# yancie-yjr/StreamYOLO

Measured on NVIDIA B200. Metric: frame-pairs/sec StreamYOLO-l 600x960 fwd+loss, higher is better.
Workload: dtype bf16

## Files before the change

include/streamyolo_sm100.h:

```cpp
#ifndef STREAMYOLO_SM100_H_
#define STREAMYOLO_SM100_H_

#include <stddef.h>
#include <stdint.h>

#ifdef __cplusplus
extern "C" {
#endif

typedef struct CUstream_st* sy_stream_t;

enum {
  SY_OK = 0,
  SY_EINVAL = 1,
  SY_EARCH = 2,
  SY_ELAUNCH = 3,
  SY_EWORKSPACE = 4
};

typedef struct {
  void* ptr;
  int32_t n, h, w, c;
  int64_t pitch;
} SyTensor;

const char* sy_last_error_string(void);
int sy_version(void);
int sy_check_device(void);

int sy_l2_persist_window(void* ptr, size_t bytes, float hit_ratio, size_t* granted, sy_stream_t stream);

enum { SY_CONV_RAW = 0, SY_CONV_FUSED = 1 };

typedef struct {
  const float* gamma; const float* beta;
  float* running_mean; float* running_var;
  int64_t* num_batches_tracked;
  int32_t c_begin;
} SyBnSegment;

typedef struct {
  SyTensor x;
  SyTensor y;
  const void* w;
  int32_t kh, kw;
  int32_t stride;
  int32_t mode;
  int32_t act;
  const float* scale;
  const float* shift;
  SyTensor res;
  int32_t split_n;
  float* stat_partials;
  int32_t n_partials;
  int32_t* rows_written;
  SyBnSegment bn[2];
  float momentum, eps;
  float* scale_shift;
  float* mean_invstd;
  uint32_t* sync;
  SyTensor apply_y, apply_res;
  int64_t apply_y_group1_offset, apply_res_group1_offset;
  void* debug_timeline;
  int32_t debug_timeline_events;
  int32_t debug_flags;
// ... 181 lines not shown
```

streamyolo_b200/csrc/conv_simt.cu:

```cuda
#include "common.cuh"

namespace sy {

struct SimtConvParams {
  const __nv_bfloat16* x; long long x_pitch;
  const __nv_bfloat16* w;
  __nv_bfloat16* y; long long y_pitch;
  const __nv_bfloat16* res; long long res_pitch;
  const float* scale; const float* shift;
  int N, H, W, Cin, Ho, Wo, Cout, kh, kw, stride, pad_h, pad_w, mode, act;
};

__global__ void conv_simt_kernel(const SimtConvParams p) {
  const int G = p.Cout / 8;
  const long long total = (long long)p.N * p.Ho * p.Wo * G;
  for (long long idx = blockIdx.x * (long long)blockDim.x + threadIdx.x; idx < total;
       idx += (long long)gridDim.x * blockDim.x) {
    const int g = (int)(idx % G);
    const long long pix = idx / G;
    const int ox = (int)(pix % p.Wo);
    const int oy = (int)((pix / p.Wo) % p.Ho);
    const int n = (int)(pix / ((long long)p.Wo * p.Ho));
    float acc[8];
#pragma unroll
// ... 95 lines not shown
    }
#pragma unroll
    for (int i = 0; i < 16; ++i) red[threadIdx.x][i] = s[i];
    __syncthreads();
    if (pl == 0 && g < G) {
      for (int i = 0; i < 16; ++i) {
        float a = 0.f;
        for (int q = 0; q < PL; ++q) a += red[q * lanes + gl][i];
        out[(i >> 3) * C + g * 8 + (i & 7)] = a;
      }
    }
    __syncthreads();
  }
}

}

using namespace sy;

extern "C" int sy_conv2d_simt(const SyConvDesc* d, sy_stream_t stream_) {
  cudaStream_t stream = reinterpret_cast<cudaStream_t>(stream_);
  SY_REQUIRE(d != nullptr, SY_EINVAL, "null descriptor");
  const SyTensor& x = d->x;
  const SyTensor& y = d->y;
  SY_REQUIRE(view_ok(x) && view_ok(y) && d->w != nullptr, SY_EINVAL, "conv2d_simt: bad x/y view or null weights");
  SY_REQUIRE((d->kh == 1 || d->kh == 3) && (d->kw == 1 || d->kw == 3) && (d->stride == 1 || d->stride == 2), SY_EINVAL,
             "conv2d_simt: kernel %dx%d stride %d unsupported", d->kh, d->kw, d->stride);
  SimtConvParams p{};
  p.pad_h = (d->kh - 1) / 2; p.pad_w = (d->kw - 1) / 2;
  p.N = x.n; p.H = x.h; p.W = x.w; p.Cin = x.c; p.Cout = y.c; p.kh = d->kh; p.kw = d->kw; p.stride = d->stride;
  p.Ho = (x.h + 2 * p.pad_h - d->kh) / d->stride + 1;
  p.Wo = (x.w + 2 * p.pad_w - d->kw) / d->stride + 1;
  SY_REQUIRE(y.n == x.n && y.h == p.Ho && y.w == p.Wo, SY_EINVAL, "conv2d_simt: output view mismatch");
  p.x = reinterpret_cast<const __nv_bfloat16*>(x.ptr); p.x_pitch = x.pitch;
  p.w = reinterpret_cast<const __nv_bfloat16*>(d->w);
  p.y = reinterpret_cast<__nv_bfloat16*>(y.ptr); p.y_pitch = y.pitch;
  p.mode = d->mode; p.act = d->act; p.scale = d->scale; p.shift = d->shift;
  if (d->mode == SY_CONV_FUSED && d->res.ptr) {
    SY_REQUIRE(view_ok(d->res) && d->res.c == y.c && d->res.h == y.h && d->res.w == y.w && d->res.n == y.n, SY_EINVAL,
               "conv2d_simt: residual view mismatch");
    p.res = reinterpret_cast<const __nv_bfloat16*>(d->res.ptr); p.res_pitch = d->res.pitch;
  }
  const long long total = (long long)p.N * p.Ho * p.Wo * (p.Cout / 8);
  const int blocks = (int)((total + 127) / 128 < 148 * 16 ? (total + 127) / 128 : 148 * 16);
  conv_simt_kernel<<<blocks, 128, 0, stream>>>(p);
  return launch_status("conv_simt_kernel");
}

extern "C" int sy_focus_pack(const float* x, int32_t b, int32_t in_ch, int32_t h, int32_t w_px, int32_t frames,
                             SyTensor y, sy_stream_t stream_) {
  cudaStream_t stream = reinterpret_cast<cudaStream_t>(stream_);
  SY_REQUIRE(x && view_ok(y), SY_EINVAL, "focus_pack: null input or bad output view");
  SY_REQUIRE(h % 2 == 0 && w_px % 2 == 0 && frames >= 1 && frames * 3 <= in_ch, SY_EINVAL,
             "focus_pack: h=%d w=%d must be even, frames=%d in_ch=%d", h, w_px, frames, in_ch);
  SY_REQUIRE(y.n == frames * b && y.h == h / 2 && y.w == w_px / 2 && y.c == 64, SY_EINVAL,
             "focus_pack: output view must be [frames*b, h/2, w/2, 64]");
  const int rows = y.n * y.h;
  const int blocks = rows < 148 * 16 ? rows : 148 * 16;
  focus_pack_kernel<<<blocks, 256, 0, stream>>>(x, b, in_ch, h, w_px, frames, reinterpret_cast<__nv_bfloat16*>(y.ptr),
                                                y.pitch);
  return launch_status("focus_pack_kernel");
}

extern "C" int sy_stats_num_partials(int32_t n, int32_t hw) { return n * cdiv(hw, kStatChunk); }

extern "C" int sy_channel_stats(SyTensor x, float* partials, int32_t n_partials, sy_stream_t stream_) {
// ... 9 lines not shown
```

streamyolo_b200/csrc/conv_tc.cu:

```cuda
#include <cuda.h>
#include <stdio.h>

#include "common.cuh"
#include "tc_common.cuh"

namespace sy {
namespace tc {

constexpr int kBlockM = 128;
constexpr int kBlockK = 64;
constexpr int kThreads = 640;
constexpr int kEpiThreads = 256;
constexpr int kTailThreads = 512;
constexpr int kABytes = kBlockM * 128;
constexpr int kMaxStages = 8;

struct BnSeg {
  const float* gamma; const float* beta;
  float* rmean; float* rvar; long long* nbt;
  int c_begin;
};

struct Params {
  int N, Ho, Wo, Cout, Cin;
  int kh, kw, stride, pad_h, pad_w;
  int th, tw, tiles_x, tiles_y;
  int m_tiles, n_tiles, total_tiles;
  FastDiv fd_m_tiles, fd_per_img, fd_tiles_x, fd_tw;
  int m_tiles2, total_tiles2;
  FastDiv fd_m_tiles2;
  int P_total;
  int gp;
  FastDiv fd_hw, fd_wo;
  int cblocks, kblocks, stages;
  int stage_tiles;
  int team;
  int stagesA;
  int halo_pitch;
  int halo_bytes;
  int halo_tx;
  int mode, act;
  __nv_bfloat16* y;
  long long y_pitch;
  const __nv_bfloat16* res;
  long long res_pitch;
  const float* scale;
  const float* shift;
  int split_n;
  float* partials;
  int n_seg;
  BnSeg seg[2];
  float momentum, eps;
  double inv_cnt[2];
  float unbias[2];
  float* ss;
  float* mi;
  unsigned int* sync;
  __nv_bfloat16* ap_y; long long ap_y_pitch;
  const __nv_bfloat16* ap_res; long long ap_res_pitch;
  long long ap_y_goff1, ap_res_goff1;
  int ap_act;
  long long* timeline;
  int timeline_cap;
  int debug_flags;
  float* dbg_f32;
};

template <bool TL>
__device__ __forceinline__ void tl_rec(const Params& p, int& n, int role, int phase, int tile, int kb) {
  if (TL && p.timeline != nullptr && blockIdx.x == 0 && n + 1 < p.timeline_cap) {
    p.timeline[2 * n] = ((long long)role << 28) | ((long long)phase << 24) | ((long long)(tile & 0xffff) << 8) | (kb & 0xff);
    p.timeline[2 * n + 1] = clock64();
    ++n;
  }
// ... 47 lines not shown
conv_tc_kernel(const __grid_constant__ CUtensorMap tmA, const __grid_constant__ CUtensorMap tmB,
               const __grid_constant__ CUtensorMap tmY, const Params p) {
  using C = Cfg<BN>;
  constexpr bool LIN = (AM == 1);
  constexpr bool HALO = (AM == 2);
  static_assert(!PAIR || AM != 0, "pair mode: linear or halo tiles");
  constexpr int kBB = PAIR ? C::kBBytes / 2 : C::kBBytes;
  const uint32_t crank = PAIR ? cluster_ctarank() : 0u;
#define SY_T_FIRST (PAIR ? (int)(blockIdx.x >> 1) : (int)blockIdx.x)
#define SY_T_STEP (PAIR ? (int)(gridDim.x >> 1) : (int)gridDim.x)
#define SY_T_END (PAIR ? p.total_tiles2 : p.total_tiles)
  auto tile_nm = [&](int tile, int& n_tile, int& m_tile) {
    if constexpr (PAIR) {
      n_tile = fdiv(tile, p.fd_m_tiles2);
      m_tile = 2 * (tile - n_tile * p.m_tiles2) + (int)crank;
    } else {
      n_tile = fdiv(tile, p.fd_m_tiles);
      m_tile = tile - n_tile * p.m_tiles;
    }
  };
  const int S = p.stages;
  constexpr int kSub = HALO ? (BN == 256 ? 1 : 3) : (PAIR ? 2 : C::kSub);
  static_assert(!PAIR || C::kSub <= 2, "pair mode: the host sizes the ring for two sub-blocks per stage");
  extern __shared__ uint8_t smem_raw[];
  uint8_t* smem = smem_raw + ((1024u - (smem_u32(smem_raw) & 1023u)) & 1023u);
  uint8_t* sA = smem;
  uint8_t* sB = sA + (HALO ? p.stagesA * p.halo_bytes : S * kSub * kABytes);
  uint8_t* sStage = sB + S * kSub * kBB;
  uint64_t* bars = reinterpret_cast<uint64_t*>(sStage + p.stage_tiles * kSlabBytes);
  const int sflip = p.stage_tiles - 1;
  uint32_t* tmem_slot = reinterpret_cast<uint32_t*>(bars + 2 * kMaxStages + 4);
  float* sAcc = reinterpret_cast<float*>(bars + 32);
  float* sScale = sAcc;
  float* sShift = sScale + 256;

  const int warp = threadIdx.x >> 5;
  const int lane = threadIdx.x & 31;
  pdl_launch_dependents();
  int tl_k = 3 * (p.timeline_cap / 4);
  if (threadIdx.x == 16 * 32) tl_rec<TL>(p, tl_k, 4, 0, 0, 0);
  const uint32_t bar0 = smem_u32(bars);
  auto full_bar = [&](int s) { return bar0 + 8u * s; };
  auto empty_bar = [&](int s) { return bar0 + 8u * (kMaxStages + s); };
  auto tfull_bar = [&](int a) { return bar0 + 8u * (2 * kMaxStages + a); };
  auto tempty_bar = [&](int a) { return bar0 + 8u * (2 * kMaxStages + 2 + a); };
  auto fullA_bar = [&](int s) { return bar0 + 8u * (2 * kMaxStages + 6 + s); };
  auto emptyA_bar = [&](int s) { return bar0 + 8u * (2 * kMaxStages + 9 + s); };

  if (threadIdx.x == 19 * 32) {
    prefetch_tmap(&tmA);
    prefetch_tmap(&tmB);
    prefetch_tmap(&tmY);
    for (int s = 0; s < S; ++s) {
      mbar_init(full_bar(s), (HALO ? 1 : 2) * (PAIR ? 2 : 1));
      mbar_init(empty_bar(s), 1);
    }
    if (HALO) {
      for (int s = 0; s < p.stagesA; ++s) {
        mbar_init(fullA_bar(s), PAIR ? 2 : 1);
        mbar_init(emptyA_bar(s), 1);
      }
    }
    for (int a = 0; a < 2; ++a) {
      mbar_init(tfull_bar(a), 1);
      mbar_init(tempty_bar(a), PAIR ? 16 : ((p.team && BN == kSlabCols) ? kEpiThreads / 2 : kEpiThreads));
    }
    fence_barrier_init();
// ... 227 lines not shown
            if (sb0 + kSub >= p.kblocks) umma_commit_2cta(tfull_bar(acc));
          } else {
            umma_commit(empty_bar(stage));
            if (sb0 + kSub >= p.kblocks) umma_commit(tfull_bar(acc));
          }
          tl_rec<TL>(p, tl_n, 1, 3, tile, sb0);
        }
        __syncwarp();
        if (++stage == S) { stage = 0; phase ^= 1u; }
      }
    }
  } else if (warp == 16) {
    const uint32_t stage_base = smem_u32(sStage);
    int sbuf = 0, prev = -1;
    int tl_s = 7 * (p.timeline_cap / 8);
    const int nbar = p.team ? 416 : 544;
    bar_free_arrive(0, nbar);
    if (sflip) bar_free_arrive(1, nbar);
    for (int tile = SY_T_FIRST; tile < SY_T_END; tile += SY_T_STEP) {
      int n_tile, m_tile;
        tile_nm(tile, n_tile, m_tile);
      int c1, c2, c3;
      if constexpr (LIN) {
        c1 = m_tile * kBlockM; c2 = 0; c3 = 0;
      } else {
        const int img = fdiv(m_tile, p.fd_per_img), rem = m_tile - img * per_img;
        const int py = fdiv(rem, p.fd_tiles_x), px = rem - py * p.tiles_x;
        c1 = px * p.tw; c2 = py * p.th; c3 = img;
      }
      for (int slab = 0; slab < BN / kSlabCols; ++slab, sbuf ^= sflip) {
        bar_staged_wait(sbuf, nbar);
        if (lane == 0) tl_rec<TL>(p, tl_s, 6, 0, tile, slab);
        if (elect_one()) {
          tma_store_4d(&tmY, stage_base + (uint32_t)(sbuf * kSlabBytes), n_tile * BN + slab * kSlabCols, c1, c2, c3);
          bulk_commit();
          if (sflip) {
            if (prev >= 0) bulk_wait_read1();
          } else {
            bulk_wait_read();
          }
        }
        __syncwarp();
        if (lane == 0) tl_rec<TL>(p, tl_s, 6, 1, tile, slab);
        if (sflip) {
          if (prev >= 0) bar_free_arrive(prev, nbar);
          prev = sbuf;
        } else {
          bar_free_arrive(0, nbar);
        }
      }
    }
    if (sflip && prev >= 0) {
      if (elect_one()) bulk_wait_read();
      __syncwarp();
      bar_free_arrive(prev, nbar);
    }
    if (lane == 0) {
      if (p.ap_y != nullptr) {
        bulk_wait_all();
        asm volatile("fence.proxy.async;" ::: "memory");
      } else {
        bulk_wait_read();
      }
    }
    __syncwarp();
    asm volatile("bar.sync 4, 288;" ::: "memory");
  } else if (warp >= 8 && warp < 16) {
    const int ew = warp - 8;
// ... 189 lines not shown
            packed[i] = valid ? pack_bf16(__uint_as_float(v[2 * i]), __uint_as_float(v[2 * i + 1])) : 0u;
          tmem_ld32(taddr + (uint32_t)(cl + 32), v);
          tl_rec<TL>(p, tl_n, 2, 2, tile, slab);
          bar_free_wait(team, 416);
#pragma unroll
          for (int g = 0; g < 4; ++g)
            sts128(my_tile_row + ((((uint32_t)g) ^ rsw) << 4), packed[4 * g], packed[4 * g + 1], packed[4 * g + 2], packed[4 * g + 3]);
          tmem_ld_wait();
          if (slab == last) {
            tcgen05_fence_before();
            mbar_arrive(tempty_bar(acc));
          }
          if (p.dbg_f32 != nullptr && valid) {
            float* o = p.dbg_f32 + pix * p.Cout + n0 + cl + 32;
#pragma unroll
            for (int i = 0; i < 32; ++i)
              if (n0 + cl + 32 + i < p.Cout) o[i] = __uint_as_float(v[i]);
          }
#pragma unroll
          for (int i = 0; i < 16; ++i)
            packed[i] = valid ? pack_bf16(__uint_as_float(v[2 * i]), __uint_as_float(v[2 * i + 1])) : 0u;
#pragma unroll
          for (int g = 0; g < 4; ++g)
            sts128(my_tile_row + ((((uint32_t)(4 + g)) ^ rsw) << 4), packed[4 * g], packed[4 * g + 1], packed[4 * g + 2], packed[4 * g + 3]);
          fence_proxy_async();
          bar_staged_arrive(team, 416);
          tl_rec<TL>(p, tl_n, 2, 3, tile, slab);
        }
      }
      tl_epi = tl_n;
      bar_free_wait(team, 416);
      asm volatile("bar.sync 4, 288;" ::: "memory");
    } else {
    for (int tile = SY_T_FIRST; tile < SY_T_END; tile += SY_T_STEP, ++it) {
      const int acc = it & 1;
      const uint32_t acc_phase = (uint32_t)(it >> 1) & 1u;
      int n_tile, m_tile;
        tile_nm(tile, n_tile, m_tile);
      bool valid;
      long long pix;
      if constexpr (LIN) {
        pix = (long long)m_tile * kBlockM + row;
        valid = pix < p.P_total;
      } else {
        const int img = fdiv(m_tile, p.fd_per_img), rem = m_tile - img * per_img;
        const int py = fdiv(rem, p.fd_tiles_x), px = rem - py * p.tiles_x;
        const int oy = py * p.th + ty, ox = px * p.tw + tx;
        valid = in_patch && (oy < p.Ho) && (ox < p.Wo);
        pix = ((long long)img * p.Ho + oy) * p.Wo + ox;
      }
      const int n0 = n_tile * BN;
      tl_rec<TL>(p, tl_n, 2, 0, tile, 0);
      if (p.mode == SY_CONV_FUSED) {
        epi_bar();
        for (int c = et; c < BN; c += kEpiThreads) {
          const int cg = n0 + c;
          sScale[c] = (cg < p.Cout && p.scale) ? p.scale[cg] : 1.0f;
          sShift[c] = (cg < p.Cout && p.shift) ? p.shift[cg] : 0.0f;
        }
        epi_bar();
      }
      mbar_wait(tfull_bar(acc), acc_phase);
      tl_rec<TL>(p, tl_n, 2, 1, tile, 0);
      tcgen05_fence_after();
      const uint32_t taddr = tmem_base + (uint32_t)(acc * BN) + ((uint32_t)(q * 32) << 16);
      const bool pf = !(p.debug_flags & 32);
      uint32_t v[32];
      tmem_ld32(taddr + (uint32_t)(half * 32), v);
#pragma unroll 1
      for (int slab = 0; slab < BN / kSlabCols; ++slab, sbuf ^= sflip) {
        const int cl = slab * kSlabCols + half * 32;
        if (!pf && slab > 0) tmem_ld32(taddr + (uint32_t)cl, v);
        tmem_ld_wait();
        if (slab == BN / kSlabCols - 1) {
          tcgen05_fence_before();
          if constexpr (PAIR) {
            __syncwarp();
            if (lane == 0) mbar_arrive_cluster(mapa(tempty_bar(acc), 0u));
          } else {
            mbar_arrive(tempty_bar(acc));
          }
        }
        if (p.dbg_f32 != nullptr && valid) {
          float* o = p.dbg_f32 + pix * p.Cout + n0 + cl;
#pragma unroll
          for (int i = 0; i < 32; ++i)
            if (n0 + cl + i < p.Cout) o[i] = __uint_as_float(v[i]);
        }
        uint32_t packed[16];
        if (p.mode == SY_CONV_RAW) {
#pragma unroll
          for (int i = 0; i < 16; ++i)
            packed[i] = valid ? pack_bf16(__uint_as_float(v[2 * i]), __uint_as_float(v[2 * i + 1])) : 0u;
        } else {
          float f[32];
#pragma unroll
          for (int i = 0; i < 32; ++i) {
            float t = __uint_as_float(v[i]) * sScale[cl + i] + sShift[cl + i];
            f[i] = p.act ? silu_f(t) : t;
          }
          if (p.res != nullptr && valid) {
            const __nv_bfloat16* rp = p.res + pix * p.res_pitch + n0 + cl;
#pragma unroll
            for (int g = 0; g < 4; ++g) {
              if (n0 + cl + g * 8 < p.Cout) {
                const uint4 rv = *reinterpret_cast<const uint4*>(rp + g * 8);
                f[g * 8 + 0] += bf16_lo(rv.x); f[g * 8 + 1] += bf16_hi(rv.x);
                f[g * 8 + 2] += bf16_lo(rv.y); f[g * 8 + 3] += bf16_hi(rv.y);
                f[g * 8 + 4] += bf16_lo(rv.z); f[g * 8 + 5] += bf16_hi(rv.z);
                f[g * 8 + 6] += bf16_lo(rv.w); f[g * 8 + 7] += bf16_hi(rv.w);
              }
            }
          }
#pragma unroll
          for (int i = 0; i < 16; ++i) packed[i] = valid ? pack_bf16(f[2 * i], f[2 * i + 1]) : 0u;
        }
        if (pf && slab + 1 < BN / kSlabCols) tmem_ld32(taddr + (uint32_t)(cl + kSlabCols), v);
        tl_rec<TL>(p, tl_n, 2, 2, tile, slab);
        bar_free_wait(sbuf);
        const uint32_t my_tile_row = my_row + (uint32_t)(sbuf * kSlabBytes);
#pragma unroll
        for (int g = 0; g < 4; ++g) {
          const uint32_t j = (uint32_t)(half * 4 + g);
          sts128(my_tile_row + ((j ^ rsw) << 4), packed[4 * g], packed[4 * g + 1], packed[4 * g + 2], packed[4 * g + 3]);
        }
        fence_proxy_async();
        bar_staged_arrive(sbuf);
        tl_rec<TL>(p, tl_n, 2, 3, tile, slab);
        tl_rec<TL>(p, tl_n, 2, 4, tile, slab);
      }
    }
    tl_epi = tl_n;
// ... 287 lines not shown

template <int BN, int AM>
static int resident_pairs(size_t smem) {
  if constexpr (AM == 0) {
    return 0;
  } else {
    static size_t seen_smem[4] = {0, 0, 0, 0};
    static int seen_n[4] = {0, 0, 0, 0};
    for (int i = 0; i < 4; ++i)
      if (seen_smem[i] == smem) return seen_n[i];
    if (!set_smem_attr<BN, AM, true>()) return 0;
    cudaLaunchConfig_t cfg = {};
    cfg.gridDim = dim3(num_sms() & ~1);
    cfg.blockDim = dim3(kThreads);
    cfg.dynamicSmemBytes = smem;
    cudaLaunchAttribute at[1];
    at[0].id = cudaLaunchAttributeClusterDimension;
    at[0].val.clusterDim.x = 2; at[0].val.clusterDim.y = 1; at[0].val.clusterDim.z = 1;
    cfg.attrs = at;
    cfg.numAttrs = 1;
    int n = 0;
    if (cudaOccupancyMaxActiveClusters(&n, conv_tc_kernel<BN, false, AM, true>, &cfg) != cudaSuccess) {
      cudaGetLastError();
      n = 0;
    }
    for (int i = 0; i < 4; ++i)
      if (seen_smem[i] == 0) { seen_smem[i] = smem; seen_n[i] = n; break; }
    return n;
  }
}

template <int BN, int AM>
static int make_plan(Params& p, Plan* out) {
  const int acc_bytes = (p.mode == SY_CONV_RAW && p.partials) ? 16 * p.Cout : 2048;
  const double kbc = BN == 256 ? 665.0 : (BN == 128 ? 515.0 : 560.0);
  const bool main_loop_bound = !(p.kblocks * kbc < epi_cycles_per_slab(BN) * (BN / 64));
  bool pair = false;
  if (AM != 0) {
    const char* e = getenv("SY_CONV_PAIR");
    const bool off = e != nullptr && e[0] == '0', force = e != nullptr && e[0] == '1';
    const char* pa = getenv("SY_PAIR_APPLY");
    const bool pair_apply = pa != nullptr && pa[0] == '1';
    pair = !off && (force || (main_loop_bound && (p.ap_y == nullptr || pair_apply)));
  }
  for (int attempt = 0; attempt < 2; ++attempt) {
    p.stage_tiles = main_loop_bound ? 1 : 2;
    if (const char* e = getenv("SY_STAGE_TILES")) p.stage_tiles = (e[0] == '2') ? 2 : 1;
    p.team = (p.stage_tiles == 2 && p.mode == SY_CONV_RAW) ? 1 : 0;
    if (const char* e = getenv("SY_CONV_TEAM")) p.team = (e[0] != '0' && p.stage_tiles == 2 && p.mode == SY_CONV_RAW) ? 1 : 0;
    if (pair) { p.stage_tiles = 1; p.team = 0; }
    const int bbytes = Cfg<BN>::kBBytes / (pair ? 2 : 1);
    const int fixed_bytes = Cfg<BN>::kFixedBytes + (p.stage_tiles - 1) * kSlabBytes;
    int smem;
    if (AM == 2) {
      const int taps = (BN == 256) ? 1 : 3;
      p.stagesA = (BN == 64 && p.cblocks > 1) ? 3 : 2;
      int stages = (kSmemLimit - fixed_bytes - acc_bytes - p.stagesA * p.halo_bytes) / (taps * bbytes);
      if (stages > kMaxStages) stages = kMaxStages;
      SY_REQUIRE(stages >= 2, SY_EINVAL, "conv2d_tc(halo): Cout=%d leaves no room for the weight ring", p.Cout);
      p.stages = stages;
      smem = fixed_bytes + acc_bytes + p.stagesA * p.halo_bytes + stages * taps * bbytes;
    } else {
      const int ksub = pair ? 2 : Cfg<BN>::kSub;
      const int stage_bytes = ksub * (kABytes + bbytes);
      int stages = (kSmemLimit - fixed_bytes - acc_bytes) / stage_bytes;
      if (stages > kMaxStages) stages = kMaxStages;
      if ((p.debug_flags >> 8) & 15) stages = min(stages, (p.debug_flags >> 8) & 15);
// ... 114 lines not shown
  tc::EncodeTiledFn enc = tc::get_encode();
  SY_REQUIRE(enc != nullptr, SY_EARCH, "cuTensorMapEncodeTiled not available from the driver");

  tc::Params p{};
  p.debug_flags = d->debug_flags;
  if (const char* e = getenv("SY_CONV_DEBUG")) p.debug_flags |= atoi(e);
  p.N = x.n; p.Ho = ho; p.Wo = wo; p.Cout = y.c; p.Cin = x.c;
  p.kh = d->kh; p.kw = d->kw; p.stride = d->stride; p.pad_h = ph; p.pad_w = pw;
  const bool halo = d->kh == 3 && d->kw == 3 && d->stride == 1 && tc::linear_tiles() &&
                    tc::use_halo(x.n, ho, wo, y.c, 9 * cdiv(x.c, tc::kBlockK));
  const bool lin = !halo && tc::linear_tiles();
  SY_REQUIRE((long long)x.n * ho * wo < (1ll << 31) - 256, SY_EINVAL, "conv2d_tc: too many output pixels");
  p.P_total = x.n * ho * wo;
  tc::pick_patch(ho, wo, &p.th, &p.tw);
  if (halo) {
    p.th = 16; p.tw = 8;
    p.halo_pitch = (p.debug_flags & 128) ? 16 : p.tw + 2;
    p.halo_tx = (p.th + 2) * p.halo_pitch * 128;
    p.halo_bytes = (p.halo_tx + 1023) / 1024 * 1024;
  }
  p.tiles_y = cdiv(ho, p.th); p.tiles_x = cdiv(wo, p.tw);
  p.m_tiles = lin ? cdiv(p.P_total, tc::kBlockM) : x.n * p.tiles_y * p.tiles_x;
  p.fd_hw = tc::make_fastdiv((uint32_t)(ho * wo));
  p.fd_wo = tc::make_fastdiv((uint32_t)wo);
  p.cblocks = cdiv(x.c, tc::kBlockK);
  p.kblocks = d->kh * d->kw * p.cblocks;
  const int bn = tc::pick_bn(y.c, halo ? cdiv(p.P_total, tc::kBlockM) : p.m_tiles, p.kblocks);
  p.n_tiles = cdiv(y.c, bn);
  p.total_tiles = p.m_tiles * p.n_tiles;
  p.fd_m_tiles = tc::make_fastdiv((uint32_t)p.m_tiles);
  p.fd_per_img = tc::make_fastdiv((uint32_t)(p.tiles_x * p.tiles_y));
  p.fd_tiles_x = tc::make_fastdiv((uint32_t)p.tiles_x);
  p.fd_tw = tc::make_fastdiv((uint32_t)p.tw);
  p.mode = d->mode; p.act = d->act;
  p.y = reinterpret_cast<__nv_bfloat16*>(y.ptr); p.y_pitch = y.pitch;
  p.res = nullptr; p.res_pitch = 0;
  if (d->mode == SY_CONV_FUSED && d->res.ptr != nullptr) {
    SY_REQUIRE(view_ok(d->res) && d->res.n == y.n && d->res.h == ho && d->res.w == wo && d->res.c == y.c, SY_EINVAL,
               "conv2d_tc: residual view mismatch");
    p.res = reinterpret_cast<const __nv_bfloat16*>(d->res.ptr); p.res_pitch = d->res.pitch;
  }
  p.scale = d->scale; p.shift = d->shift;
  p.split_n = (d->split_n > 0 && d->split_n < x.n) ? d->split_n : x.n;
  p.gp = p.split_n * ho * wo;
  p.partials = (d->mode == SY_CONV_RAW) ? d->stat_partials : nullptr;
  if (p.partials) {
    SY_REQUIRE(((uintptr_t)p.partials % 16) == 0, SY_EINVAL, "conv2d_tc: statistic rows not 16B aligned");
    SY_REQUIRE(d->n_partials >= tc::num_sms(), SY_EWORKSPACE, "conv2d_tc: %d statistic rows, need %d (sy_conv_stat_rows)",
               d->n_partials, tc::num_sms());
  }
  p.dbg_f32 = d->debug_f32;
  p.timeline = reinterpret_cast<long long*>(d->debug_timeline);
  p.timeline_cap = d->debug_timeline ? d->debug_timeline_events : 0;
  p.n_seg = 0;
  if (p.partials && d->bn[0].gamma != nullptr) {
    SY_REQUIRE(d->sync && d->scale_shift, SY_EINVAL, "conv2d_tc: BN finalize needs sync counters and scale_shift");
    for (int sgi = 0; sgi < 2; ++sgi) {
      if (d->bn[sgi].gamma == nullptr) break;
      SY_REQUIRE(d->bn[sgi].beta != nullptr && d->bn[sgi].c_begin >= 0 && d->bn[sgi].c_begin < y.c, SY_EINVAL,
                 "conv2d_tc: bad BN segment %d", sgi);
      p.seg[sgi].gamma = d->bn[sgi].gamma; p.seg[sgi].beta = d->bn[sgi].beta;
      p.seg[sgi].rmean = d->bn[sgi].running_mean; p.seg[sgi].rvar = d->bn[sgi].running_var;
      p.seg[sgi].nbt = reinterpret_cast<long long*>(d->bn[sgi].num_batches_tracked);
      p.seg[sgi].c_begin = d->bn[sgi].c_begin;
      p.n_seg = sgi + 1;
    }
    SY_REQUIRE(p.seg[0].c_begin == 0, SY_EINVAL, "conv2d_tc: first BN segment must start at channel 0");
    p.momentum = d->momentum; p.eps = d->eps;
    {
      const int groups = p.split_n < x.n ? 2 : 1;
      for (int g = 0; g < 2; ++g) {
        const double cnt = (double)(g == 0 ? (groups == 2 ? p.split_n : x.n) : x.n - p.split_n) * ho * wo;
        p.inv_cnt[g] = cnt > 0.0 ? 1.0 / cnt : 0.0;
        p.unbias[g] = cnt > 1.0 ? (float)(cnt / (cnt - 1.0)) : 1.0f;
      }
    }
    p.ss = d->scale_shift;
    p.mi = d->mean_invstd;
// ... 123 lines not shown
```

streamyolo_b200/csrc/dwconv.cu:

```cuda
#include "common.cuh"

namespace sy {

struct DwParams {
  const __nv_bfloat16* x; long long x_pitch;
  const __nv_bfloat16* w;
  __nv_bfloat16* y; long long y_pitch;
  const __nv_bfloat16* res; long long res_pitch;
  const float* scale; const float* shift;
  int N, H, W, C, Ho, Wo, k, stride, pad, mode, act;
};

template <int K>
__global__ void __launch_bounds__(256) dwconv_kernel(const DwParams p) {
  const int G = p.C >> 3;
  const long long total = (long long)p.N * p.Ho * p.Wo * G;
  for (long long idx = blockIdx.x * (long long)blockDim.x + threadIdx.x; idx < total; idx += (long long)gridDim.x * blockDim.x) {
    const int g = (int)(idx % G);
    const long long pix = idx / G;
    const int ox = (int)(pix % p.Wo), oy = (int)((pix / p.Wo) % p.Ho);
    const int n = (int)(pix / ((long long)p.Wo * p.Ho));
    float acc[8] = {0.f, 0.f, 0.f, 0.f, 0.f, 0.f, 0.f, 0.f};
#pragma unroll
    for (int r = 0; r < K; ++r) {
// ... 16 lines not shown
      for (int i = 0; i < 8; ++i) {
        const int c = g * 8 + i;
        const float t = acc[i] * (p.scale ? p.scale[c] : 1.f) + (p.shift ? p.shift[c] : 0.f);
        acc[i] = p.act ? silu_f(t) : t;
      }
      if (p.res != nullptr) {
        const uint4 rv = *reinterpret_cast<const uint4*>(p.res + pix * p.res_pitch + g * 8);
        acc[0] += bf16_lo(rv.x); acc[1] += bf16_hi(rv.x); acc[2] += bf16_lo(rv.y); acc[3] += bf16_hi(rv.y);
        acc[4] += bf16_lo(rv.z); acc[5] += bf16_hi(rv.z); acc[6] += bf16_lo(rv.w); acc[7] += bf16_hi(rv.w);
      }
    }
    *reinterpret_cast<uint4*>(p.y + pix * p.y_pitch + g * 8) =
        make_uint4(pack_bf16(acc[0], acc[1]), pack_bf16(acc[2], acc[3]), pack_bf16(acc[4], acc[5]), pack_bf16(acc[6], acc[7]));
  }
}

}

using namespace sy;

extern "C" int sy_dwconv2d(const SyConvDesc* d, sy_stream_t stream_) {
  cudaStream_t stream = reinterpret_cast<cudaStream_t>(stream_);
  SY_REQUIRE(d != nullptr, SY_EINVAL, "null descriptor");
  const SyTensor& x = d->x;
  const SyTensor& y = d->y;
  SY_REQUIRE(view_ok(x) && view_ok(y) && d->w != nullptr, SY_EINVAL, "dwconv2d: bad x/y view or null weights");
  SY_REQUIRE(d->kh == d->kw && (d->kh == 1 || d->kh == 3 || d->kh == 5) && (d->stride == 1 || d->stride == 2), SY_EINVAL,
             "dwconv2d: kernel %dx%d stride %d unsupported", d->kh, d->kw, d->stride);
  const int pad = (d->kh - 1) / 2;
  const int ho = (x.h + 2 * pad - d->kh) / d->stride + 1, wo = (x.w + 2 * pad - d->kw) / d->stride + 1;
  SY_REQUIRE(y.n == x.n && y.h == ho && y.w == wo && y.c == x.c, SY_EINVAL, "dwconv2d: output view %dx%dx%dx%d, expected %dx%dx%dx%d",
             y.n, y.h, y.w, y.c, x.n, ho, wo, x.c);
  SY_REQUIRE(((uintptr_t)d->w % 16) == 0, SY_EINVAL, "dwconv2d: weights not 16B aligned");
  DwParams p{};
  p.x = reinterpret_cast<const __nv_bfloat16*>(x.ptr); p.x_pitch = x.pitch;
  p.w = reinterpret_cast<const __nv_bfloat16*>(d->w);
  p.y = reinterpret_cast<__nv_bfloat16*>(y.ptr); p.y_pitch = y.pitch;
  p.res = nullptr;
  if (d->mode == SY_CONV_FUSED && d->res.ptr != nullptr) {
    SY_REQUIRE(view_ok(d->res) && d->res.n == y.n && d->res.h == ho && d->res.w == wo && d->res.c == y.c, SY_EINVAL,
               "dwconv2d: residual view mismatch");
    p.res = reinterpret_cast<const __nv_bfloat16*>(d->res.ptr); p.res_pitch = d->res.pitch;
  }
  p.scale = d->scale; p.shift = d->shift;
  p.N = x.n; p.H = x.h; p.W = x.w; p.C = x.c; p.Ho = ho; p.Wo = wo; p.k = d->kh; p.stride = d->stride; p.pad = pad;
  p.mode = d->mode; p.act = d->act;
  const long long total = (long long)x.n * ho * wo * (x.c / 8);
  long long blocks = (total + 255) / 256;
  if (blocks > 148ll * 32) blocks = 148ll * 32;
  if (blocks < 1) blocks = 1;
  switch (d->kh) {
    case 1: dwconv_kernel<1><<<(int)blocks, 256, 0, stream>>>(p); break;
    case 3: dwconv_kernel<3><<<(int)blocks, 256, 0, stream>>>(p); break;
    default: dwconv_kernel<5><<<(int)blocks, 256, 0, stream>>>(p); break;
  }
  return launch_status("dwconv_kernel");
}
```

streamyolo_b200/model/engine.py:

```python
import os

import torch

from .. import ops
from ..ops import View


FUSE_APPLY = os.environ.get("SY_FUSE_APPLY", "0") != "0"
FUSE_APPLY_MAX_BYTES = float(os.environ.get("SY_FUSE_APPLY_MAX_MB", "0")) * 1e6
WEIGHT_EPOCH = 0
TRACE = None


def name_modules(model):
    for n, m in model.named_modules():
        m._sy_name = n


def _trace(m, y):
    if TRACE is not None:
        TRACE[getattr(m, "_sy_name", str(id(m)))] = y.torch().permute(0, 3, 1, 2).float().cpu()


class Ctx:
# ... 108 lines not shown
            return View.empty(n, h, w, c, ctx.device)
        arena = torch.empty(int(RAW_ARENA_MB * 1e6) // 256 * 256, dtype=torch.uint8, device=ctx.device)
        st = _RAW_ARENAS[key] = [arena, ops.l2_persist_window(arena)]
    return View(st[0][:nbytes].view(torch.bfloat16).view(n, h, w, c))


def _arm_raw_window(device):
    st = _RAW_ARENAS.get(str(device))
    if st is not None and st[1] > 0 and not torch.cuda.is_current_stream_capturing():
        ops.l2_persist_window(st[0])


_CAPTURE_STREAMS = {}


def graph_capture_stream(device):
    key = str(device)
    if key not in _CAPTURE_STREAMS:
        _CAPTURE_STREAMS[key] = torch.cuda.Stream(device=device)
    st = _CAPTURE_STREAMS[key]
    with torch.cuda.stream(st):
        _arm_raw_window(device)
    return st


def _dbg_skip_apply(nbytes):
    e = os.environ.get("SY_DBG_SKIP_APPLY")
    if not e:
        return False
    lo, hi = (float(v) for v in e.split(":"))
    return lo * 1e6 <= nbytes < hi * 1e6


def conv_bn_act(ctx: Ctx, mods, x: View, wpk, k, s, y: View, res: View = None, act=1, y_goff1=0, res_goff1=0, impl=None):
    kh, kw = (k, k) if isinstance(k, int) else k
    ho = (x.h + 2 * ((kh - 1) // 2) - kh) // s + 1
    wo = (x.w + 2 * ((kw - 1) // 2) - kw) // s + 1
    cout = sum(m.conv.out_channels for m in mods)
    raw = _raw_view(ctx, x.n, ho, wo, cout)
    bn0 = mods[0].bn
    mom = float(0.1 if bn0.momentum is None else bn0.momentum)
    n = x.n
    split = ctx.split if ctx.groups == 2 else 0
    for m in mods:
        m._stats_epoch = getattr(m, "_stats_epoch", 0) + 1
    impl = impl or ctx.impl
    if impl == "tc":
        partials = torch.empty((ops.conv_stat_rows(), 4 * cout), dtype=torch.float32, device=ctx.device)
        segs, c0 = [], 0
        for m in mods:
            segs.append(_bn_seg(m, c0))
            c0 += m.conv.out_channels
        ss = torch.empty((2, 2, cout), dtype=torch.float32, device=ctx.device)
        if FUSE_APPLY or n * ho * wo * cout * 2 <= FUSE_APPLY_MAX_BYTES:
            ops.conv2d(x, wpk, raw, k, s, ops.SY_CONV_RAW, impl="tc", partials=partials, split_n=split, bn=segs,
                       momentum=mom, eps=float(bn0.eps), scale_shift=ss, sync=_sync(mods[0], ctx.device), act=act,
                       apply_y=y, apply_res=res, y_goff1=y_goff1, res_goff1=res_goff1)
        else:
            ops.conv2d(x, wpk, raw, k, s, ops.SY_CONV_RAW, impl="tc", partials=partials, split_n=split, bn=segs,
                       momentum=mom, eps=float(bn0.eps), scale_shift=ss, sync=_sync(mods[0], ctx.device))
            if not _dbg_skip_apply(n * ho * wo * cout * 2):
                ops.bn_act_apply(raw, ss[0].data_ptr(), ss[1].data_ptr(), split if split else n, act, res, y, y_goff1,
                                 res_goff1)
        return
    ops.conv2d(x, wpk, raw, k, s, ops.SY_CONV_RAW, impl=impl)
    sc = torch.empty((2, 2, cout), dtype=torch.float32, device=ctx.device)
    sp = split if split else n
    c0 = 0
    for m in mods:
        c = m.conv.out_channels
        P = ops.stats_num_partials(n, ho * wo)
        partials = torch.empty((P, 2, c), dtype=torch.float32, device=ctx.device)
        ops.channel_stats(raw.ch(c0, c), partials)
        tmp = torch.empty((2, 2, c), dtype=torch.float32, device=ctx.device)
        bn = m.bn
        ops.bn_finalize(partials, (P // n) * sp if split else 0, 2 if split else 1, sp * ho * wo,
                        bn.weight, bn.bias, bn.running_mean, bn.running_var, bn.num_batches_tracked,
                        mom, float(bn.eps), tmp[0], tmp[1])
        sc[:, :, c0:c0 + c] = tmp
        c0 += c
    if y_goff1 == 0 and res_goff1 == 0:
        ops.bn_act_apply(raw, sc[0], sc[1], sp, act, res, y)
    else:
        nb = sp
        ops.bn_act_apply(raw.imgs(0, nb), sc[0, 0], sc[1, 0], nb, act,
                         res.imgs(0, nb) if res is not None else None, y.imgs(0, nb))
        y1 = View(y.buf, y.c0, y.c, y.n0, nb).shifted(y_goff1 + nb * y.img_elems())
        r1 = View(res.buf, res.c0, res.c, res.n0, nb).shifted(res_goff1 + nb * res.img_elems()) if res is not None else None
        ops.bn_act_apply(raw.imgs(nb, nb), sc[0, 1], sc[1, 1], nb, act, r1, y1)


def base_conv(ctx: Ctx, m, x: View, y: View = None, res: View = None) -> View:
    if hasattr(m, "dconv"):
        return base_conv(ctx, m.pconv, base_conv(ctx, m.dconv, x), y, res)
    k, s = m.ksize, m.stride
    ho, wo = ops.conv_out_hw(x.h, x.w, k, s)
    cout = m.conv.out_channels
# ... 194 lines not shown
```

streamyolo_b200/ops.py:

```python
import ctypes as C
import os

import torch

_HERE = os.path.dirname(os.path.abspath(__file__))
LIB_PATH = os.path.join(_HERE, "lib", "libstreamyolo_sm100.so")

SY_CONV_RAW, SY_CONV_FUSED = 0, 1


class SyTensor(C.Structure):
    _fields_ = [("ptr", C.c_void_p), ("n", C.c_int32), ("h", C.c_int32), ("w", C.c_int32), ("c", C.c_int32),
                ("pitch", C.c_int64)]


class SyBnSegment(C.Structure):
    _fields_ = [("gamma", C.c_void_p), ("beta", C.c_void_p), ("running_mean", C.c_void_p),
                ("running_var", C.c_void_p), ("num_batches_tracked", C.c_void_p), ("c_begin", C.c_int32)]


class SyConvDesc(C.Structure):
    _fields_ = [("x", SyTensor), ("y", SyTensor), ("w", C.c_void_p), ("kh", C.c_int32), ("kw", C.c_int32),
                ("stride", C.c_int32), ("mode", C.c_int32), ("act", C.c_int32), ("scale", C.c_void_p),
                ("shift", C.c_void_p), ("res", SyTensor), ("split_n", C.c_int32), ("stat_partials", C.c_void_p),
                ("n_partials", C.c_int32), ("rows_written", C.POINTER(C.c_int32)), ("bn", SyBnSegment * 2),
                ("momentum", C.c_float), ("eps", C.c_float), ("scale_shift", C.c_void_p), ("mean_invstd", C.c_void_p),
                ("sync", C.c_void_p),
                ("apply_y", SyTensor), ("apply_res", SyTensor), ("apply_y_group1_offset", C.c_int64),
                ("apply_res_group1_offset", C.c_int64),
                ("debug_timeline", C.c_void_p),
                ("debug_timeline_events", C.c_int32), ("debug_flags", C.c_int32), ("debug_f32", C.c_void_p)]


class SyHeadPredDesc(C.Structure):
    _fields_ = [("cls_feat", SyTensor), ("reg_feat", SyTensor),
                ("w_reg", C.c_void_p), ("b_reg", C.c_void_p), ("w_obj", C.c_void_p), ("b_obj", C.c_void_p),
                ("w_cls", C.c_void_p), ("b_cls", C.c_void_p),
                ("num_classes", C.c_int32), ("stride", C.c_int32), ("anchor_offset", C.c_int32),
                ("a_total", C.c_int32), ("sigmoid", C.c_int32), ("decode", C.c_int32),
                ("out", C.c_void_p), ("origin", C.c_void_p)]

# ... 225 lines not shown
    _, i, kh, kw = ws[0].shape
    out = torch.empty((sum(w.shape[0] for w in ws), kh * kw, i), dtype=torch.bfloat16, device=ws[0].device)
    o0 = 0
    for w in ws:
        w = _w32(w)
        assert tuple(w.shape[1:]) == (i, kh, kw)
        _check(lib().sy_pack_conv_weight(w.data_ptr(), w.shape[0], i, kh, kw, 0, out.data_ptr() + 2 * o0 * kh * kw * i, 0, 0,
                                         _stream()))
        o0 += w.shape[0]
    return out


def conv_out_hw(h, w, k, s):
    p = (k - 1) // 2
    return (h + 2 * p - k) // s + 1, (w + 2 * p - k) // s + 1


def conv_stat_rows():
    return load_library().sy_conv_stat_rows()


def conv2d(x: View, wpk, y: View, k, s, mode, impl="tc", scale=None, shift=None, act=1, res: View = None,
           partials=None, split_n=0, timeline=None, debug_flags=0, bn=None, momentum=0.03, eps=1e-3, scale_shift=None,
           sync=None, apply_y: View = None, apply_res: View = None, y_goff1=0, res_goff1=0, mean_invstd=None, debug_f32=None):
    d = SyConvDesc()
    d.x, d.y = x.st(), y.st()
    d.w = wpk.data_ptr()
    d.kh, d.kw = (k, k) if isinstance(k, int) else k
    d.stride, d.mode, d.act = s, mode, act
    d.scale = scale.data_ptr() if scale is not None else None
    d.shift = shift.data_ptr() if shift is not None else None
    d.res = res.st() if res is not None else NULL_T
    d.split_n = split_n
    rows = C.c_int32(0)
    if partials is not None:
        d.stat_partials, d.n_partials = partials.data_ptr(), partials.shape[0]
        d.rows_written = C.pointer(rows)
    if bn:
        for i, (g, b_, rm, rv, nbt, c0) in enumerate(bn):
            seg = d.bn[i]
            seg.gamma, seg.beta = g.data_ptr(), b_.data_ptr()
            seg.running_mean = rm.data_ptr() if rm is not None else None
            seg.running_var = rv.data_ptr() if rv is not None else None
            seg.num_batches_tracked = nbt.data_ptr() if nbt is not None else None
            seg.c_begin = c0
        d.momentum, d.eps = momentum, eps
        d.scale_shift, d.sync = scale_shift.data_ptr(), sync.data_ptr()
        d.mean_invstd = mean_invstd.data_ptr() if mean_invstd is not None else None
        if apply_y is not None:
            d.apply_y = apply_y.st()
            d.apply_res = apply_res.st() if apply_res is not None else NULL_T
            d.apply_y_group1_offset, d.apply_res_group1_offset = y_goff1, res_goff1
    d.debug_flags = debug_flags
    d.debug_f32 = debug_f32.data_ptr() if debug_f32 is not None else None
    if timeline is not None:
        d.debug_timeline, d.debug_timeline_events = timeline.data_ptr(), timeline.numel() // 2
    fn = {"tc": lib().sy_conv2d_tc, "simt": lib().sy_conv2d_simt, "dw": lib().sy_dwconv2d}[impl]
    _check(fn(C.byref(d), _stream()))
    return rows.value


def focus_pack(x, frames, y: View):
    assert x.dtype == torch.float32 and x.is_contiguous()
    b, ch, h, w = x.shape
    _check(lib().sy_focus_pack(x.data_ptr(), b, ch, h, w, frames, y.st(), _stream()))


STEM_K = (3, 1)


def pack_dw_weight(w):
    c, one, kh, kw = w.shape
    assert one == 1
    return pack_conv_weight(_w32(w).view(1, c, kh, kw)).view(kh * kw, c)


def pack_stem_weight(w):
    w = _w32(w)
    o, i, kh, kw = w.shape
    out = torch.empty((o, kh, 64), dtype=torch.bfloat16, device=w.device)
# ... 263 lines not shown
```

Before: 1473.

## Recompute cheap convs for BN instead of storing raw activations

Adds two tensor-core conv modes: a stats-only pass that accumulates BN statistics without storing output, and a BN-apply pass that recomputes the conv and applies per-group scale/shift and activation in the epilogue. For stride-1 convs with small reduction depth whose raw output exceeds the raw arena, the engine runs conv twice rather than writing and rereading a large raw bf16 tensor. This trades extra MMA work for less HBM traffic and one fewer elementwise kernel. The apply pass rounds the accumulator to bf16 first so it matches the stored-raw path.

After: 1424, median of 6. -3.3%, worse.

```diff
diff --git a/include/streamyolo_sm100.h b/include/streamyolo_sm100.h
--- a/include/streamyolo_sm100.h
+++ b/include/streamyolo_sm100.h
@@ -30,7 +30,7 @@
 
 int sy_l2_persist_window(void* ptr, size_t bytes, float hit_ratio, size_t* granted, sy_stream_t stream);
 
-enum { SY_CONV_RAW = 0, SY_CONV_FUSED = 1 };
+enum { SY_CONV_RAW = 0, SY_CONV_FUSED = 1, SY_CONV_STATS = 2, SY_CONV_BN_APPLY = 3 };
 
 typedef struct {
   const float* gamma; const float* beta;
diff --git a/streamyolo_b200/csrc/conv_simt.cu b/streamyolo_b200/csrc/conv_simt.cu
--- a/streamyolo_b200/csrc/conv_simt.cu
+++ b/streamyolo_b200/csrc/conv_simt.cu
@@ -151,6 +151,7 @@
   p.Ho = (x.h + 2 * p.pad_h - d->kh) / d->stride + 1;
   p.Wo = (x.w + 2 * p.pad_w - d->kw) / d->stride + 1;
   SY_REQUIRE(y.n == x.n && y.h == p.Ho && y.w == p.Wo, SY_EINVAL, "conv2d_simt: output view mismatch");
+  SY_REQUIRE(d->mode == SY_CONV_RAW || d->mode == SY_CONV_FUSED, SY_EINVAL, "conv2d_simt: mode %d is tensor-core only", d->mode);
   p.x = reinterpret_cast<const __nv_bfloat16*>(x.ptr); p.x_pitch = x.pitch;
   p.w = reinterpret_cast<const __nv_bfloat16*>(d->w);
   p.y = reinterpret_cast<__nv_bfloat16*>(y.ptr); p.y_pitch = y.pitch;
diff --git a/streamyolo_b200/csrc/conv_tc.cu b/streamyolo_b200/csrc/conv_tc.cu
--- a/streamyolo_b200/csrc/conv_tc.cu
+++ b/streamyolo_b200/csrc/conv_tc.cu
@@ -40,6 +40,8 @@
   int halo_bytes;
   int halo_tx;
   int mode, act;
+  int store;
+  int bn_apply;
   __nv_bfloat16* y;
   long long y_pitch;
   const __nv_bfloat16* res;
@@ -153,7 +155,7 @@
   uint32_t* tmem_slot = reinterpret_cast<uint32_t*>(bars + 2 * kMaxStages + 4);
   float* sAcc = reinterpret_cast<float*>(bars + 32);
   float* sScale = sAcc;
-  float* sShift = sScale + 256;
+  float* sShift = sScale + (p.bn_apply ? 512 : 256);
 
   const int warp = threadIdx.x >> 5;
   const int lane = threadIdx.x & 31;
@@ -447,8 +449,10 @@
         bar_staged_wait(sbuf, nbar);
         if (lane == 0) tl_rec<TL>(p, tl_s, 6, 0, tile, slab);
         if (elect_one()) {
-          tma_store_4d(&tmY, stage_base + (uint32_t)(sbuf * kSlabBytes), n_tile * BN + slab * kSlabCols, c1, c2, c3);
-          bulk_commit();
+          if (p.store) {
+            tma_store_4d(&tmY, stage_base + (uint32_t)(sbuf * kSlabBytes), n_tile * BN + slab * kSlabCols, c1, c2, c3);
+            bulk_commit();
+          }
           if (sflip) {
             if (prev >= 0) bulk_wait_read1();
           } else {
@@ -704,6 +708,7 @@
       bar_free_wait(team, 416);
       asm volatile("bar.sync 4, 288;" ::: "memory");
     } else {
+    int sc_n0 = -1;
     for (int tile = SY_T_FIRST; tile < SY_T_END; tile += SY_T_STEP, ++it) {
       const int acc = it & 1;
       const uint32_t acc_phase = (uint32_t)(it >> 1) & 1u;
@@ -723,14 +728,23 @@
       }
       const int n0 = n_tile * BN;
       tl_rec<TL>(p, tl_n, 2, 0, tile, 0);
-      if (p.mode == SY_CONV_FUSED) {
+      if (p.mode == SY_CONV_FUSED && n0 != sc_n0) {
         epi_bar();
-        for (int c = et; c < BN; c += kEpiThreads) {
-          const int cg = n0 + c;
-          sScale[c] = (cg < p.Cout && p.scale) ? p.scale[cg] : 1.0f;
-          sShift[c] = (cg < p.Cout && p.shift) ? p.shift[cg] : 0.0f;
+        if (p.bn_apply) {
+          for (int i = et; i < 2 * BN; i += kEpiThreads) {
+            const int g = i / BN, c = i - g * BN, cg = n0 + c;
+            sScale[g * 256 + c] = cg < p.Cout ? p.ss[g * p.Cout + cg] : 1.0f;
+            sShift[g * 256 + c] = cg < p.Cout ? p.ss[(2 + g) * p.Cout + cg] : 0.0f;
+          }
+        } else {
+          for (int c = et; c < BN; c += kEpiThreads) {
+            const int cg = n0 + c;
+            sScale[c] = (cg < p.Cout && p.scale) ? p.scale[cg] : 1.0f;
+            sShift[c] = (cg < p.Cout && p.shift) ? p.shift[cg] : 0.0f;
+          }
         }
         epi_bar();
+        sc_n0 = n0;
       }
       mbar_wait(tfull_bar(acc), acc_phase);
       tl_rec<TL>(p, tl_n, 2, 1, tile, 0);
@@ -766,10 +780,20 @@
             packed[i] = valid ? pack_bf16(__uint_as_float(v[2 * i]), __uint_as_float(v[2 * i + 1])) : 0u;
         } else {
           float f[32];
-#pragma unroll
-          for (int i = 0; i < 32; ++i) {
-            float t = __uint_as_float(v[i]) * sScale[cl + i] + sShift[cl + i];
-            f[i] = p.act ? silu_f(t) : t;
+          if (p.bn_apply) {
+            const float* scg = sScale + ((pix >= p.gp) ? 256 : 0);
+            const float* shg = sShift + ((pix >= p.gp) ? 256 : 0);
+#pragma unroll
+            for (int i = 0; i < 32; ++i) {
+              const float t = __bfloat162float(__float2bfloat16_rn(__uint_as_float(v[i]))) * scg[cl + i] + shg[cl + i];
+              f[i] = p.act ? silu_f(t) : t;
+            }
+          } else {
+#pragma unroll
+            for (int i = 0; i < 32; ++i) {
+              float t = __uint_as_float(v[i]) * sScale[cl + i] + sShift[cl + i];
+              f[i] = p.act ? silu_f(t) : t;
+            }
           }
           if (p.res != nullptr && valid) {
             const __nv_bfloat16* rp = p.res + pix * p.res_pitch + n0 + cl;
@@ -1123,7 +1147,7 @@
 
 template <int BN, int AM>
 static int make_plan(Params& p, Plan* out) {
-  const int acc_bytes = (p.mode == SY_CONV_RAW && p.partials) ? 16 * p.Cout : 2048;
+  const int acc_bytes = (p.mode == SY_CONV_RAW && p.partials) ? 16 * p.Cout : (p.bn_apply ? 4096 : 2048);
   const double kbc = BN == 256 ? 665.0 : (BN == 128 ? 515.0 : 560.0);
   const bool main_loop_bound = !(p.kblocks * kbc < epi_cycles_per_slab(BN) * (BN / 64));
   bool pair = false;
@@ -1304,10 +1328,16 @@
   p.fd_per_img = tc::make_fastdiv((uint32_t)(p.tiles_x * p.tiles_y));
   p.fd_tiles_x = tc::make_fastdiv((uint32_t)p.tiles_x);
   p.fd_tw = tc::make_fastdiv((uint32_t)p.tw);
-  p.mode = d->mode; p.act = d->act;
+  SY_REQUIRE(d->mode >= SY_CONV_RAW && d->mode <= SY_CONV_BN_APPLY, SY_EINVAL, "conv2d_tc: unknown mode %d", d->mode);
+  const bool stats_only = d->mode == SY_CONV_STATS, bn_apply = d->mode == SY_CONV_BN_APPLY;
+  p.mode = stats_only ? SY_CONV_RAW : (bn_apply ? SY_CONV_FUSED : d->mode);
+  p.store = stats_only ? 0 : 1;
+  p.bn_apply = bn_apply ? 1 : 0;
+  p.act = d->act;
   p.y = reinterpret_cast<__nv_bfloat16*>(y.ptr); p.y_pitch = y.pitch;
   p.res = nullptr; p.res_pitch = 0;
-  if (d->mode == SY_CONV_FUSED && d->res.ptr != nullptr) {
+  SY_REQUIRE(!bn_apply || d->res.ptr == nullptr, SY_EINVAL, "conv2d_tc(bn_apply): no residual");
+  if (p.mode == SY_CONV_FUSED && d->res.ptr != nullptr) {
     SY_REQUIRE(view_ok(d->res) && d->res.n == y.n && d->res.h == ho && d->res.w == wo && d->res.c == y.c, SY_EINVAL,
                "conv2d_tc: residual view mismatch");
     p.res = reinterpret_cast<const __nv_bfloat16*>(d->res.ptr); p.res_pitch = d->res.pitch;
@@ -1315,7 +1345,14 @@
   p.scale = d->scale; p.shift = d->shift;
   p.split_n = (d->split_n > 0 && d->split_n < x.n) ? d->split_n : x.n;
   p.gp = p.split_n * ho * wo;
-  p.partials = (d->mode == SY_CONV_RAW) ? d->stat_partials : nullptr;
+  p.partials = (p.mode == SY_CONV_RAW) ? d->stat_partials : nullptr;
+  if (stats_only)
+    SY_REQUIRE(d->stat_partials != nullptr && d->bn[0].gamma != nullptr && d->apply_y.ptr == nullptr, SY_EINVAL,
+               "conv2d_tc(stats): needs stat_partials and bn[], and stores nothing");
+  if (bn_apply) {
+    SY_REQUIRE(d->scale_shift != nullptr, SY_EINVAL, "conv2d_tc(bn_apply): needs scale_shift");
+    p.ss = d->scale_shift;
+  }
   if (p.partials) {
     SY_REQUIRE(((uintptr_t)p.partials % 16) == 0, SY_EINVAL, "conv2d_tc: statistic rows not 16B aligned");
     SY_REQUIRE(d->n_partials >= tc::num_sms(), SY_EWORKSPACE, "conv2d_tc: %d statistic rows, need %d (sy_conv_stat_rows)",
diff --git a/streamyolo_b200/csrc/dwconv.cu b/streamyolo_b200/csrc/dwconv.cu
--- a/streamyolo_b200/csrc/dwconv.cu
+++ b/streamyolo_b200/csrc/dwconv.cu
@@ -72,6 +72,7 @@
   SY_REQUIRE(y.n == x.n && y.h == ho && y.w == wo && y.c == x.c, SY_EINVAL, "dwconv2d: output view %dx%dx%dx%d, expected %dx%dx%dx%d",
              y.n, y.h, y.w, y.c, x.n, ho, wo, x.c);
   SY_REQUIRE(((uintptr_t)d->w % 16) == 0, SY_EINVAL, "dwconv2d: weights not 16B aligned");
+  SY_REQUIRE(d->mode == SY_CONV_RAW || d->mode == SY_CONV_FUSED, SY_EINVAL, "dwconv2d: mode %d is tensor-core only", d->mode);
   DwParams p{};
   p.x = reinterpret_cast<const __nv_bfloat16*>(x.ptr); p.x_pitch = x.pitch;
   p.w = reinterpret_cast<const __nv_bfloat16*>(d->w);
diff --git a/streamyolo_b200/model/engine.py b/streamyolo_b200/model/engine.py
--- a/streamyolo_b200/model/engine.py
+++ b/streamyolo_b200/model/engine.py
@@ -164,12 +164,20 @@
     return lo * 1e6 <= nbytes < hi * 1e6
 
 
+RECOMPUTE_BN = True
+RECOMPUTE_MAX_K = 192
+
+
+def recompute_bn(n, ho, wo, cin, cout, kh, kw, s):
+    return (s == 1 and cin <= cout and kh * kw * cin <= RECOMPUTE_MAX_K
+            and n * ho * wo * cout * 2 > RAW_ARENA_MB * 1e6)
+
+
 def conv_bn_act(ctx: Ctx, mods, x: View, wpk, k, s, y: View, res: View = None, act=1, y_goff1=0, res_goff1=0, impl=None):
     kh, kw = (k, k) if isinstance(k, int) else k
     ho = (x.h + 2 * ((kh - 1) // 2) - kh) // s + 1
     wo = (x.w + 2 * ((kw - 1) // 2) - kw) // s + 1
     cout = sum(m.conv.out_channels for m in mods)
-    raw = _raw_view(ctx, x.n, ho, wo, cout)
     bn0 = mods[0].bn
     mom = float(0.1 if bn0.momentum is None else bn0.momentum)
     n = x.n
@@ -184,6 +192,13 @@
             segs.append(_bn_seg(m, c0))
             c0 += m.conv.out_channels
         ss = torch.empty((2, 2, cout), dtype=torch.float32, device=ctx.device)
+        if (RECOMPUTE_BN and not FUSE_APPLY and res is None and y_goff1 == 0
+                and recompute_bn(n, ho, wo, x.c, cout, kh, kw, s)):
+            ops.conv2d(x, wpk, y, k, s, ops.SY_CONV_STATS, impl="tc", partials=partials, split_n=split, bn=segs,
+                       momentum=mom, eps=float(bn0.eps), scale_shift=ss, sync=_sync(mods[0], ctx.device))
+            ops.conv2d(x, wpk, y, k, s, ops.SY_CONV_BN_APPLY, impl="tc", split_n=split, scale_shift=ss, act=act)
+            return
+        raw = _raw_view(ctx, x.n, ho, wo, cout)
         if FUSE_APPLY or n * ho * wo * cout * 2 <= FUSE_APPLY_MAX_BYTES:
             ops.conv2d(x, wpk, raw, k, s, ops.SY_CONV_RAW, impl="tc", partials=partials, split_n=split, bn=segs,
                        momentum=mom, eps=float(bn0.eps), scale_shift=ss, sync=_sync(mods[0], ctx.device), act=act,
@@ -195,6 +210,7 @@
                 ops.bn_act_apply(raw, ss[0].data_ptr(), ss[1].data_ptr(), split if split else n, act, res, y, y_goff1,
                                  res_goff1)
         return
+    raw = _raw_view(ctx, x.n, ho, wo, cout)
     ops.conv2d(x, wpk, raw, k, s, ops.SY_CONV_RAW, impl=impl)
     sc = torch.empty((2, 2, cout), dtype=torch.float32, device=ctx.device)
     sp = split if split else n
diff --git a/streamyolo_b200/ops.py b/streamyolo_b200/ops.py
--- a/streamyolo_b200/ops.py
+++ b/streamyolo_b200/ops.py
@@ -6,7 +6,7 @@
 _HERE = os.path.dirname(os.path.abspath(__file__))
 LIB_PATH = os.path.join(_HERE, "lib", "libstreamyolo_sm100.so")
 
-SY_CONV_RAW, SY_CONV_FUSED = 0, 1
+SY_CONV_RAW, SY_CONV_FUSED, SY_CONV_STATS, SY_CONV_BN_APPLY = 0, 1, 2, 3
 
 
 class SyTensor(C.Structure):
@@ -298,6 +298,7 @@
     d.shift = shift.data_ptr() if shift is not None else None
     d.res = res.st() if res is not None else NULL_T
     d.split_n = split_n
+    d.scale_shift = scale_shift.data_ptr() if scale_shift is not None else None
     rows = C.c_int32(0)
     if partials is not None:
         d.stat_partials, d.n_partials = partials.data_ptr(), partials.shape[0]
@@ -311,7 +312,7 @@
             seg.num_batches_tracked = nbt.data_ptr() if nbt is not None else None
             seg.c_begin = c0
         d.momentum, d.eps = momentum, eps
-        d.scale_shift, d.sync = scale_shift.data_ptr(), sync.data_ptr()
+        d.sync = sync.data_ptr()
         d.mean_invstd = mean_invstd.data_ptr() if mean_invstd is not None else None
         if apply_y is not None:
             d.apply_y = apply_y.st()
```
